# naver/dust3r

Measured on NVIDIA H100. Metric: image-pairs/sec (512x384, ViT-L/B+DPT), higher is better.
Workload: dtype bf16

## Files before the change

dust3r_b200/csrc/attention_wgmma.cu:

```cuda
#include "d3r_common.cuh"
#include "sm90_ptx.cuh"
#include "elementwise.h"
#include "prof.h"
#include "pdl.cuh"

namespace d3r {
namespace attn {

namespace wg {

constexpr int BQ = 128, BK = 128, D = 64;
constexpr int kThreads = 384;
constexpr int kTileBytes = 128 * 64 * 2;
constexpr int kPBytes = 2 * 64 * 128 * 2;
template <bool P_SMEM>
struct Smem {
  static constexpr int kP = P_SMEM ? 2 * kPBytes : 0;
  static constexpr int kBytes = kTileBytes  + 2 * kTileBytes  + 2 * kTileBytes  + kP + 128  + 1024;
  static_assert(kBytes <= 227 * 1024, "shared memory of one CTA");
};

template <bool P_SMEM>
__global__ void __launch_bounds__(kThreads, 1)
attention_kernel(const __grid_constant__ CUtensorMap tmap_q, const __grid_constant__ CUtensorMap tmap_k,
                 const __grid_constant__ CUtensorMap tmap_v, __nv_bfloat16* __restrict__ out, long long ldo, int Nq, int Nk,
                 int heads, int total_tiles, float scale_log2) {
  extern __shared__ uint8_t smem_raw[];
  uint8_t* smem = reinterpret_cast<uint8_t*>((reinterpret_cast<uintptr_t>(smem_raw) + 1023) & ~uintptr_t(1023));
  uint8_t* s_q = smem;
  uint8_t* s_k = s_q + kTileBytes;
  uint8_t* s_v = s_k + 2 * kTileBytes;
  uint8_t* s_p = s_v + 2 * kTileBytes;
  uint64_t* bars = reinterpret_cast<uint64_t*>(s_p + Smem<P_SMEM>::kP);
  uint64_t* q_full = bars + 0;
  uint64_t* q_empty = bars + 1;
  uint64_t* k_full = bars + 2;
  uint64_t* k_empty = bars + 4;
  uint64_t* v_full = bars + 6;
  uint64_t* v_empty = bars + 8;

  const int warp = threadIdx.x >> 5, lane = threadIdx.x & 31;
  const int nq_tiles = (Nq + BQ - 1) / BQ;
  const int nblk = (Nk + BK - 1) / BK;
  auto tile_coords = [&](int t, int& q0, int& h, int& b) {
    q0 = (t % nq_tiles) * BQ;
    h = (t / nq_tiles) % heads;
    b = t / (nq_tiles * heads);
  };

  if (threadIdx.x == 0) {
    ptx::prefetch_tmap(&tmap_q);
    ptx::prefetch_tmap(&tmap_k);
    ptx::prefetch_tmap(&tmap_v);
    ptx::mbar_init(ptx::smem_u32(q_full), 1);
    ptx::mbar_init(ptx::smem_u32(q_empty), 8);
    for (int s = 0; s < 2; ++s) {
      ptx::mbar_init(ptx::smem_u32(&k_full[s]), 1);
      ptx::mbar_init(ptx::smem_u32(&k_empty[s]), 8);
      ptx::mbar_init(ptx::smem_u32(&v_full[s]), 1);
      ptx::mbar_init(ptx::smem_u32(&v_empty[s]), 8);
    }
    ptx::fence_barrier_init();
  }
  __syncthreads();
  pdl::sync_with_predecessor();

  if (warp < 4) {
    ptx::setmaxnreg_dec<24>();
    if (warp == 0 && ptx::elect_one()) {
      uint32_t g = 0, it = 0;
      for (int t = blockIdx.x; t < total_tiles; t += gridDim.x, ++it) {
        int q0, h, b;
        tile_coords(t, q0, h, b);
        ptx::mbar_wait(ptx::smem_u32(q_empty), (it & 1) ^ 1);
        ptx::mbar_arrive_expect_tx(ptx::smem_u32(q_full), kTileBytes);
        ptx::tma_load_3d(ptx::smem_u32(s_q), &tmap_q, ptx::smem_u32(q_full), h * D, q0, b);
        for (int j = 0; j < nblk; ++j, ++g) {
          const int st = g & 1;
          const uint32_t ph = (g >> 1) & 1;
          ptx::mbar_wait(ptx::smem_u32(&k_empty[st]), ph ^ 1);
          ptx::mbar_arrive_expect_tx(ptx::smem_u32(&k_full[st]), kTileBytes);
          ptx::tma_load_3d(ptx::smem_u32(s_k + st * kTileBytes), &tmap_k, ptx::smem_u32(&k_full[st]), h * D, j * BK, b);
          ptx::mbar_wait(ptx::smem_u32(&v_empty[st]), ph ^ 1);
          ptx::mbar_arrive_expect_tx(ptx::smem_u32(&v_full[st]), kTileBytes);
          ptx::tma_load_3d(ptx::smem_u32(s_v + st * kTileBytes), &tmap_v, ptx::smem_u32(&v_full[st]), h * D, j * BK, b);
        }
      }
    }
  } else {
    ptx::setmaxnreg_inc<240>();
    const int cw = (threadIdx.x >> 7) - 1;
    const int wq = warp & 3, q = lane & 3;
    uint8_t* s_pw = s_p + cw * kPBytes;
    uint32_t g = 0, it = 0;
    for (int t = blockIdx.x; t < total_tiles; t += gridDim.x, ++it) {
      int q0, h, b;
      tile_coords(t, q0, h, b);
      float m_run[2] = {-INFINITY, -INFINITY}, l_run[2] = {0.f, 0.f};
      float o[32];
#pragma unroll
      for (int i = 0; i < 32; ++i) o[i] = 0.f;
      ptx::mbar_wait(ptx::smem_u32(q_full), it & 1);
      const uint64_t dq = ptx::desc_kmajor_sw128(ptx::smem_u32(s_q + cw * 64 * 128));
      for (int j = 0; j < nblk; ++j, ++g) {
        const int st = g & 1;
        const uint32_t ph = (g >> 1) & 1;
        float s[64];
        ptx::mbar_wait(ptx::smem_u32(&k_full[st]), ph);
        const uint64_t dk = ptx::desc_kmajor_sw128(ptx::smem_u32(s_k + st * kTileBytes));
        ptx::wgmma_fence();
#pragma unroll
        for (int k = 0; k < D / 16; ++k) ptx::wgmma_m64n128k16_ss(s, dq + uint64_t(2 * k), dk + uint64_t(2 * k), k ? 1u : 0u);
        ptx::wgmma_commit();
        ptx::wgmma_wait<0>();
        ptx::reg_fence(s);
        if (lane == 0) {
          ptx::mbar_arrive(ptx::smem_u32(&k_empty[st]));
          if (j == nblk - 1) ptx::mbar_arrive(ptx::smem_u32(q_empty));
        }
        const int nvalid = Nk - j * BK;
        if (nvalid < BK) {
#pragma unroll
          for (int n = 0; n < 16; ++n)
#pragma unroll
            for (int e = 0; e < 2; ++e)
              if (8 * n + 2 * q + e >= nvalid) { s[4 * n + e] = -INFINITY; s[4 * n + 2 + e] = -INFINITY; }
        }
        float ms[2];
#pragma unroll
        for (int hh = 0; hh < 2; ++hh) {
          float mx = -INFINITY;
#pragma unroll
          for (int n = 0; n < 16; ++n) mx = fmaxf(mx, fmaxf(s[4 * n + 2 * hh], s[4 * n + 2 * hh + 1]));
          mx = fmaxf(mx, __shfl_xor_sync(0xffffffffu, mx, 1));
          mx = fmaxf(mx, __shfl_xor_sync(0xffffffffu, mx, 2));
          const float m_new = fmaxf(m_run[hh], mx);
          const float corr = ptx::ex2_approx((m_run[hh] - m_new) * scale_log2);
          m_run[hh] = m_new;
          l_run[hh] *= corr;
#pragma unroll
          for (int n = 0; n < 8; ++n) { o[4 * n + 2 * hh] *= corr; o[4 * n + 2 * hh + 1] *= corr; }
          ms[hh] = m_new * scale_log2;
        }
        uint32_t pk[32];
#pragma unroll
        for (int n = 0; n < 16; ++n)
#pragma unroll
          for (int hh = 0; hh < 2; ++hh) {
            const float p0 = ptx::ex2_approx(fmaf(s[4 * n + 2 * hh], scale_log2, -ms[hh]));
            const float p1 = ptx::ex2_approx(fmaf(s[4 * n + 2 * hh + 1], scale_log2, -ms[hh]));
            l_run[hh] += p0 + p1;
            pk[2 * n + hh] = pack_bf16x2(p0, p1);
          }
        ptx::mbar_wait(ptx::smem_u32(&v_full[st]), ph);
        const uint32_t sv = ptx::smem_u32(s_v + st * kTileBytes);
        if constexpr (P_SMEM) {
#pragma unroll
          for (int n = 0; n < 16; ++n)
#pragma unroll
            for (int hh = 0; hh < 2; ++hh) {
              const int r = wq * 16 + (lane >> 2) + 8 * hh;
              *reinterpret_cast<uint32_t*>(s_pw + (n >> 3) * (64 * 128) + r * 128 + (((n & 7) ^ (r & 7)) << 4) + 4 * q) = pk[2 * n + hh];
            }
          ptx::fence_proxy_async();
          asm volatile("bar.sync %0, 128;" ::"r"(1 + cw) : "memory");
          const uint32_t sp = ptx::smem_u32(s_pw);
          ptx::wgmma_fence();
#pragma unroll
          for (int kk = 0; kk < BK / 16; ++kk)
            ptx::wgmma_m64n64k16_ss_tb(o, ptx::desc_kmajor_sw128(sp + (kk >> 2) * (64 * 128)) + uint64_t(2 * (kk & 3)),
                                       ptx::desc_mnmajor_sw128(sv + kk * 16 * 128), 1u);
        } else {
          ptx::wgmma_fence();
#pragma unroll
          for (int kk = 0; kk < BK / 16; ++kk) ptx::wgmma_m64n64k16_rs_tb(o, pk + 4 * kk, ptx::desc_mnmajor_sw128(sv + kk * 16 * 128), 1u);
        }
        ptx::wgmma_commit();
        ptx::wgmma_wait<0>();
        ptx::reg_fence(o);
        if constexpr (P_SMEM) asm volatile("bar.sync %0, 128;" ::"r"(1 + cw) : "memory");
        if (lane == 0) ptx::mbar_arrive(ptx::smem_u32(&v_empty[st]));
      }
#pragma unroll
      for (int hh = 0; hh < 2; ++hh) {
        float l = l_run[hh];
        l += __shfl_xor_sync(0xffffffffu, l, 1);
        l += __shfl_xor_sync(0xffffffffu, l, 2);
        const float inv = 1.f / l;
        const int qrow = q0 + cw * 64 + wq * 16 + (lane >> 2) + 8 * hh;
        if (qrow < Nq) {
          __nv_bfloat16* orow = out + ((long long)b * Nq + qrow) * ldo + h * D + 2 * q;
#pragma unroll
          for (int n = 0; n < 8; ++n)
            *reinterpret_cast<uint32_t*>(orow + 8 * n) = pack_bf16x2(o[4 * n + 2 * hh] * inv, o[4 * n + 2 * hh + 1] * inv);
        }
      }
    }
  }
}

}

template <bool P_SMEM>
static int launch_attention(const CUtensorMap& mq, const CUtensorMap& mk, const CUtensorMap& mv, void* out, long long ldo, int B, int heads,
                            int Nq, int Nk, float scale, cudaStream_t st) {
  static unsigned long long attr_devices = 0;
  if (first_launch_on_this_device(attr_devices))
    D3R_CUDA(cudaFuncSetAttribute(wg::attention_kernel<P_SMEM>, cudaFuncAttributeMaxDynamicSharedMemorySize, wg::Smem<P_SMEM>::kBytes));
  const int total_tiles = ((Nq + wg::BQ - 1) / wg::BQ) * heads * B;
  const int slots = num_sms();
  const int rounds = (total_tiles + slots - 1) / slots;
  const int grid = (total_tiles + rounds - 1) / rounds;
  prof::Scope scope(P_SMEM ? "attention_wgmma_psmem" : "attention_wgmma", st, 4.0 * double(B) * heads * double(Nq) * double(Nk) * 64.0);
  D3R_CUDA(pdl::launch(wg::attention_kernel<P_SMEM>, dim3(grid), dim3(wg::kThreads), size_t(wg::Smem<P_SMEM>::kBytes), st, mq, mk, mv,
                       (__nv_bfloat16*)out, ldo, Nq, Nk, heads, total_tiles, scale * 1.4426950408889634f));
  D3R_LAUNCH_CHECK();
  return D3R_OK;
}

static int make_map(CUtensorMap* m, const void* base, long long ld, int cols, int N, int B, int box_rows) {
  const cuuint64_t dims[3] = {(cuuint64_t)cols, (cuuint64_t)N, (cuuint64_t)B};
  const cuuint64_t str[2] = {(cuuint64_t)ld * 2, (cuuint64_t)N * ld * 2};
  const cuuint32_t box[3] = {64, (cuuint32_t)box_rows, 1};
  return encode_tensor_map(m, base, 3, dims, str, box, "attention");
}

static int g_impl = 3;

int attention_hd64(const void* q, long long ldq, const void* k, long long ldk, const void* v, long long ldv, void* out,
                   long long ldo, int B, int heads, int Nq, int Nk, float scale, cudaStream_t st) {
  D3R_CHECK_ARG(q && k && v && out && B > 0 && heads > 0 && Nq > 0 && Nk > 0, "attention: bad arguments");
  D3R_CHECK_ARG(ldq % 8 == 0 && ldk % 8 == 0 && ldv % 8 == 0 && ldo % 8 == 0, "attention: row strides must be multiples of 8");
  D3R_CHECK_ARG(((uintptr_t)q & 15) == 0 && ((uintptr_t)k & 15) == 0 && ((uintptr_t)v & 15) == 0 && ((uintptr_t)out & 15) == 0,
                "attention: pointers must be 16-byte aligned");
  CUtensorMap mq, mk, mv;
  int rc;
  if ((rc = make_map(&mq, q, ldq, heads * 64, Nq, B, wg::BQ))) return rc;
  if ((rc = make_map(&mk, k, ldk, heads * 64, Nk, B, wg::BK))) return rc;
  if ((rc = make_map(&mv, v, ldv, heads * 64, Nk, B, wg::BK))) return rc;
  if (g_impl == 2) return launch_attention<true>(mq, mk, mv, out, ldo, B, heads, Nq, Nk, scale, st);
  return launch_attention<false>(mq, mk, mv, out, ldo, B, heads, Nq, Nk, scale, st);
}

}
}

extern "C" void d3r_set_attention_impl(int32_t impl) { d3r::attn::g_impl = (impl == 2) ? 2 : 3; }

extern "C" int d3r_attention_hd64(const void* q, int64_t ldq, const void* k, int64_t ldk, const void* v, int64_t ldv, void* out,
                                  int64_t ldo, int32_t B, int32_t heads, int32_t Nq, int32_t Nk, float scale, void* stream) {
  return d3r::attn::attention_hd64(q, ldq, k, ldk, v, ldv, out, ldo, B, heads, Nq, Nk, scale, (cudaStream_t)stream);
}
```

dust3r_b200/csrc/sm90_ptx.cuh:

```cuda
#pragma once
#include <cuda.h>
#include <cuda_runtime.h>
#include <cuda_bf16.h>
#include <cstdint>

namespace d3r {
namespace ptx {

__device__ __forceinline__ uint32_t smem_u32(const void* p) { return static_cast<uint32_t>(__cvta_generic_to_shared(p)); }

__device__ __forceinline__ bool elect_one() {
  uint32_t pred = 0;
  asm volatile(
      "{\n"
      ".reg .b32 %%rx;\n"
      ".reg .pred %%px;\n"
      "elect.sync %%rx|%%px, %1;\n"
      "@%%px mov.s32 %0, 1;\n"
      "}\n"
      : "+r"(pred)
      : "r"(0xffffffffu));
  return pred != 0;
}

__device__ __forceinline__ void mbar_init(uint32_t bar, uint32_t count) {
  asm volatile("mbarrier.init.shared::cta.b64 [%0], %1;" ::"r"(bar), "r"(count));
}
__device__ __forceinline__ void fence_barrier_init() { asm volatile("fence.mbarrier_init.release.cluster;" ::: "memory"); }
__device__ __forceinline__ void fence_proxy_async() { asm volatile("fence.proxy.async.shared::cta;" ::: "memory"); }

__device__ __forceinline__ void mbar_arrive_expect_tx(uint32_t bar, uint32_t bytes) {
  asm volatile("mbarrier.arrive.expect_tx.shared::cta.b64 _, [%0], %1;" ::"r"(bar), "r"(bytes) : "memory");
}
__device__ __forceinline__ void mbar_arrive(uint32_t bar) {
  asm volatile("mbarrier.arrive.shared::cta.b64 _, [%0];" ::"r"(bar) : "memory");
}
__device__ __forceinline__ bool mbar_try_wait(uint32_t bar, uint32_t parity) {
  uint32_t done;
  asm volatile(
      "{\n"
      ".reg .pred p;\n"
      "mbarrier.try_wait.parity.shared::cta.b64 p, [%1], %2;\n"
      "selp.u32 %0, 1, 0, p;\n"
      "}\n"
      : "=r"(done)
      : "r"(bar), "r"(parity)
      : "memory");
  return done != 0;
}
__device__ __forceinline__ void mbar_wait(uint32_t bar, uint32_t parity) {
  while (!mbar_try_wait(bar, parity)) {
  }
}
__device__ __forceinline__ void mbar_wait_bounded(uint32_t bar, uint32_t parity) {
  uint32_t spins = 0;
  bool done;
  do {
    done = mbar_try_wait(bar, parity);
    if (!done && ++spins > (1u << 22)) __trap();
  } while (!done);
}

__device__ __forceinline__ void bulk_g2s(uint32_t dst, const void* src, uint32_t bytes, uint32_t bar) {
  asm volatile("cp.async.bulk.shared::cluster.global.mbarrier::complete_tx::bytes [%0], [%1], %2, [%3];"
               ::"r"(dst), "l"(src), "r"(bytes), "r"(bar) : "memory");
}
__device__ __forceinline__ uint64_t policy_evict_first() {
  uint64_t pol;
  asm volatile("createpolicy.fractional.L2::evict_first.b64 %0, 1.0;" : "=l"(pol));
  return pol;
}
__device__ __forceinline__ void bulk_g2s_hint(uint32_t dst, const void* src, uint32_t bytes, uint32_t bar, uint64_t pol) {
  asm volatile("cp.async.bulk.shared::cluster.global.mbarrier::complete_tx::bytes.L2::cache_hint [%0], [%1], %2, [%3], %4;"
               ::"r"(dst), "l"(src), "r"(bytes), "r"(bar), "l"(pol) : "memory");
}

__device__ __forceinline__ void prefetch_tmap(const void* tmap) {
  asm volatile("prefetch.tensormap [%0];" ::"l"(reinterpret_cast<uint64_t>(tmap)) : "memory");
}
__device__ __forceinline__ void tma_load_2d(uint32_t dst, const void* tmap, uint32_t bar, int c0, int c1) {
  asm volatile(
      "cp.async.bulk.tensor.2d.shared::cluster.global.mbarrier::complete_tx::bytes [%0], [%1, {%3, %4}], [%2];"
      ::"r"(dst), "l"(reinterpret_cast<uint64_t>(tmap)), "r"(bar), "r"(c0), "r"(c1)
      : "memory");
}
__device__ __forceinline__ void tma_load_3d(uint32_t dst, const void* tmap, uint32_t bar, int c0, int c1, int c2) {
  asm volatile(
      "cp.async.bulk.tensor.3d.shared::cluster.global.mbarrier::complete_tx::bytes [%0], [%1, {%3, %4, %5}], [%2];"
      ::"r"(dst), "l"(reinterpret_cast<uint64_t>(tmap)), "r"(bar), "r"(c0), "r"(c1), "r"(c2)
      : "memory");
}
__device__ __forceinline__ void tma_load_4d(uint32_t dst, const void* tmap, uint32_t bar, int c0, int c1, int c2, int c3) {
  asm volatile(
      "cp.async.bulk.tensor.4d.shared::cluster.global.mbarrier::complete_tx::bytes [%0], [%1, {%3, %4, %5, %6}], [%2];"
      ::"r"(dst), "l"(reinterpret_cast<uint64_t>(tmap)), "r"(bar), "r"(c0), "r"(c1), "r"(c2), "r"(c3)
      : "memory");
}
__device__ __forceinline__ void tma_load_3d_mc(uint32_t dst, const void* tmap, uint32_t bar, int c0, int c1, int c2, uint16_t mask) {
  asm volatile(
      "cp.async.bulk.tensor.3d.shared::cluster.global.mbarrier::complete_tx::bytes.multicast::cluster [%0], [%1, {%3, %4, %5}], [%2], %6;"
      ::"r"(dst), "l"(reinterpret_cast<uint64_t>(tmap)), "r"(bar), "r"(c0), "r"(c1), "r"(c2), "h"(mask)
      : "memory");
}

__device__ __forceinline__ void tma_store_2d(const void* tmap, uint32_t src, int c0, int c1) {
  asm volatile("cp.async.bulk.tensor.2d.global.shared::cta.tile.bulk_group [%0, {%2, %3}], [%1];"
               ::"l"(reinterpret_cast<uint64_t>(tmap)), "r"(src), "r"(c0), "r"(c1) : "memory");
}
__device__ __forceinline__ void tma_store_4d(const void* tmap, uint32_t src, int c0, int c1, int c2, int c3) {
  asm volatile("cp.async.bulk.tensor.4d.global.shared::cta.tile.bulk_group [%0, {%2, %3, %4, %5}], [%1];"
               ::"l"(reinterpret_cast<uint64_t>(tmap)), "r"(src), "r"(c0), "r"(c1), "r"(c2), "r"(c3) : "memory");
}
__device__ __forceinline__ void tma_reduce_add_2d(const void* tmap, uint32_t src, int c0, int c1) {
  asm volatile("cp.reduce.async.bulk.tensor.2d.global.shared::cta.add.tile.bulk_group [%0, {%2, %3}], [%1];"
               ::"l"(reinterpret_cast<uint64_t>(tmap)), "r"(src), "r"(c0), "r"(c1) : "memory");
}
__device__ __forceinline__ void bulk_commit_group() { asm volatile("cp.async.bulk.commit_group;" ::: "memory"); }
template <int N> __device__ __forceinline__ void bulk_wait_group_read() { asm volatile("cp.async.bulk.wait_group.read %0;" ::"n"(N) : "memory"); }
template <int N> __device__ __forceinline__ void bulk_wait_group() { asm volatile("cp.async.bulk.wait_group %0;" ::"n"(N) : "memory"); }
__device__ __forceinline__ void st_shared_b32(uint32_t addr, uint32_t v) { asm volatile("st.shared.b32 [%0], %1;" ::"r"(addr), "r"(v) : "memory"); }
__device__ __forceinline__ uint32_t ld_shared_b32(uint32_t addr) {
  uint32_t v;
  asm volatile("ld.shared.b32 %0, [%1];" : "=r"(v) : "r"(addr) : "memory");
  return v;
}
__device__ __forceinline__ void st_shared_v2_f32(uint32_t addr, float a, float b) {
  asm volatile("st.shared.v2.f32 [%0], {%1, %2};" ::"r"(addr), "f"(a), "f"(b) : "memory");
}
__device__ __forceinline__ void named_bar_sync(uint32_t id, uint32_t count) { asm volatile("bar.sync %0, %1;" ::"r"(id), "r"(count) : "memory"); }

__device__ __forceinline__ uint32_t cluster_ctarank() {
  uint32_t r;
  asm volatile("mov.u32 %0, %%cluster_ctarank;" : "=r"(r));
  return r;
}
__device__ __forceinline__ void cluster_sync() {
  asm volatile("barrier.cluster.arrive.release.aligned;\nbarrier.cluster.wait.acquire.aligned;" ::: "memory");
}
__device__ __forceinline__ void mbar_arrive_cluster(uint32_t bar, uint32_t rank) {
  asm volatile(
      "{\n"
      ".reg .b32 raddr;\n"
      "mapa.shared::cluster.u32 raddr, %0, %1;\n"
      "mbarrier.arrive.shared::cluster.b64 _, [raddr];\n"
      "}\n" ::"r"(bar), "r"(rank) : "memory");
}

__device__ __forceinline__ float ex2_approx(float x) { float y; asm("ex2.approx.ftz.f32 %0, %1;" : "=f"(y) : "f"(x)); return y; }
__device__ __forceinline__ float rcp_approx(float x) { float y; asm("rcp.approx.ftz.f32 %0, %1;" : "=f"(y) : "f"(x)); return y; }
__device__ __forceinline__ float rsqrt_approx(float x) { float y; asm("rsqrt.approx.ftz.f32 %0, %1;" : "=f"(y) : "f"(x)); return y; }
__device__ __forceinline__ float sqrt_approx(float x) { float y; asm("sqrt.approx.ftz.f32 %0, %1;" : "=f"(y) : "f"(x)); return y; }

template <int N> __device__ __forceinline__ void setmaxnreg_dec() { asm volatile("setmaxnreg.dec.sync.aligned.u32 %0;" ::"n"(N)); }
template <int N> __device__ __forceinline__ void setmaxnreg_inc() { asm volatile("setmaxnreg.inc.sync.aligned.u32 %0;" ::"n"(N)); }

__device__ __forceinline__ void wgmma_fence() { asm volatile("wgmma.fence.sync.aligned;" ::: "memory"); }
__device__ __forceinline__ void wgmma_commit() { asm volatile("wgmma.commit_group.sync.aligned;" ::: "memory"); }
template <int N> __device__ __forceinline__ void wgmma_wait() { asm volatile("wgmma.wait_group.sync.aligned %0;" ::"n"(N) : "memory"); }
template <int N> __device__ __forceinline__ void reg_fence(float (&d)[N]) {
#pragma unroll
  for (int i = 0; i < N; ++i) asm volatile("" : "+f"(d[i])::"memory");
}

__device__ __forceinline__ uint64_t desc_sw128(uint32_t smem_addr, uint32_t lbo_bytes) {
  uint64_t d = 0;
  d |= uint64_t((smem_addr & 0x3FFFF) >> 4);
  d |= uint64_t(lbo_bytes >> 4) << 16;
  d |= uint64_t(1024 >> 4) << 32;
  d |= uint64_t(1) << 62;
  return d;
}
__device__ __forceinline__ uint64_t desc_kmajor_sw128(uint32_t smem_addr) { return desc_sw128(smem_addr, 16); }
__device__ __forceinline__ uint64_t desc_mnmajor_sw128(uint32_t smem_addr) { return desc_sw128(smem_addr, 1024); }

__device__ __forceinline__ void wgmma_m64n64k16_ss(float* d, uint64_t desc_a, uint64_t desc_b, uint32_t accumulate) {
  asm volatile(
      "{\n"
      ".reg .pred p;\n"
      "setp.ne.b32 p, %34, 0;\n"
      "wgmma.mma_async.sync.aligned.m64n64k16.f32.bf16.bf16 "
      "{%0, %1, %2, %3, %4, %5, %6, %7, %8, %9, %10, %11, %12, %13, %14, %15, %16, %17, %18, %19, %20, %21, %22, %23, %24, %25, %26, %27, %28, %29, %30, %31}, %32, %33, p, 1, 1, 0, 0;\n"
      "}\n"
      : "+f"(d[0]), "+f"(d[1]), "+f"(d[2]), "+f"(d[3]), "+f"(d[4]), "+f"(d[5]), "+f"(d[6]), "+f"(d[7]), "+f"(d[8]), "+f"(d[9]), "+f"(d[10]), "+f"(d[11]), "+f"(d[12]), "+f"(d[13]), "+f"(d[14]), "+f"(d[15]), "+f"(d[16]), "+f"(d[17]), "+f"(d[18]), "+f"(d[19]), "+f"(d[20]), "+f"(d[21]), "+f"(d[22]), "+f"(d[23]), "+f"(d[24]), "+f"(d[25]), "+f"(d[26]), "+f"(d[27]), "+f"(d[28]), "+f"(d[29]), "+f"(d[30]), "+f"(d[31])
      : "l"(desc_a), "l"(desc_b), "r"(accumulate));
}
__device__ __forceinline__ void wgmma_m64n128k16_ss(float* d, uint64_t desc_a, uint64_t desc_b, uint32_t accumulate) {
  asm volatile(
      "{\n"
      ".reg .pred p;\n"
      "setp.ne.b32 p, %66, 0;\n"
      "wgmma.mma_async.sync.aligned.m64n128k16.f32.bf16.bf16 "
      "{%0, %1, %2, %3, %4, %5, %6, %7, %8, %9, %10, %11, %12, %13, %14, %15, %16, %17, %18, %19, %20, %21, %22, %23, %24, %25, %26, %27, %28, %29, %30, %31, %32, %33, %34, %35, %36, %37, %38, %39, %40, %41, %42, %43, %44, %45, %46, %47, %48, %49, %50, %51, %52, %53, %54, %55, %56, %57, %58, %59, %60, %61, %62, %63}, %64, %65, p, 1, 1, 0, 0;\n"
      "}\n"
      : "+f"(d[0]), "+f"(d[1]), "+f"(d[2]), "+f"(d[3]), "+f"(d[4]), "+f"(d[5]), "+f"(d[6]), "+f"(d[7]), "+f"(d[8]), "+f"(d[9]), "+f"(d[10]), "+f"(d[11]), "+f"(d[12]), "+f"(d[13]), "+f"(d[14]), "+f"(d[15]), "+f"(d[16]), "+f"(d[17]), "+f"(d[18]), "+f"(d[19]), "+f"(d[20]), "+f"(d[21]), "+f"(d[22]), "+f"(d[23]), "+f"(d[24]), "+f"(d[25]), "+f"(d[26]), "+f"(d[27]), "+f"(d[28]), "+f"(d[29]), "+f"(d[30]), "+f"(d[31]), "+f"(d[32]), "+f"(d[33]), "+f"(d[34]), "+f"(d[35]), "+f"(d[36]), "+f"(d[37]), "+f"(d[38]), "+f"(d[39]), "+f"(d[40]), "+f"(d[41]), "+f"(d[42]), "+f"(d[43]), "+f"(d[44]), "+f"(d[45]), "+f"(d[46]), "+f"(d[47]), "+f"(d[48]), "+f"(d[49]), "+f"(d[50]), "+f"(d[51]), "+f"(d[52]), "+f"(d[53]), "+f"(d[54]), "+f"(d[55]), "+f"(d[56]), "+f"(d[57]), "+f"(d[58]), "+f"(d[59]), "+f"(d[60]), "+f"(d[61]), "+f"(d[62]), "+f"(d[63])
      : "l"(desc_a), "l"(desc_b), "r"(accumulate));
}
__device__ __forceinline__ void wgmma_m64n256k16_ss(float* d, uint64_t desc_a, uint64_t desc_b, uint32_t accumulate) {
  asm volatile(
      "{\n"
      ".reg .pred p;\n"
      "setp.ne.b32 p, %130, 0;\n"
      "wgmma.mma_async.sync.aligned.m64n256k16.f32.bf16.bf16 "
      "{%0, %1, %2, %3, %4, %5, %6, %7, %8, %9, %10, %11, %12, %13, %14, %15, %16, %17, %18, %19, %20, %21, %22, %23, %24, %25, %26, %27, %28, %29, %30, %31, %32, %33, %34, %35, %36, %37, %38, %39, %40, %41, %42, %43, %44, %45, %46, %47, %48, %49, %50, %51, %52, %53, %54, %55, %56, %57, %58, %59, %60, %61, %62, %63, %64, %65, %66, %67, %68, %69, %70, %71, %72, %73, %74, %75, %76, %77, %78, %79, %80, %81, %82, %83, %84, %85, %86, %87, %88, %89, %90, %91, %92, %93, %94, %95, %96, %97, %98, %99, %100, %101, %102, %103, %104, %105, %106, %107, %108, %109, %110, %111, %112, %113, %114, %115, %116, %117, %118, %119, %120, %121, %122, %123, %124, %125, %126, %127}, %128, %129, p, 1, 1, 0, 0;\n"
      "}\n"
      : "+f"(d[0]), "+f"(d[1]), "+f"(d[2]), "+f"(d[3]), "+f"(d[4]), "+f"(d[5]), "+f"(d[6]), "+f"(d[7]), "+f"(d[8]), "+f"(d[9]), "+f"(d[10]), "+f"(d[11]), "+f"(d[12]), "+f"(d[13]), "+f"(d[14]), "+f"(d[15]), "+f"(d[16]), "+f"(d[17]), "+f"(d[18]), "+f"(d[19]), "+f"(d[20]), "+f"(d[21]), "+f"(d[22]), "+f"(d[23]), "+f"(d[24]), "+f"(d[25]), "+f"(d[26]), "+f"(d[27]), "+f"(d[28]), "+f"(d[29]), "+f"(d[30]), "+f"(d[31]), "+f"(d[32]), "+f"(d[33]), "+f"(d[34]), "+f"(d[35]), "+f"(d[36]), "+f"(d[37]), "+f"(d[38]), "+f"(d[39]), "+f"(d[40]), "+f"(d[41]), "+f"(d[42]), "+f"(d[43]), "+f"(d[44]), "+f"(d[45]), "+f"(d[46]), "+f"(d[47]), "+f"(d[48]), "+f"(d[49]), "+f"(d[50]), "+f"(d[51]), "+f"(d[52]), "+f"(d[53]), "+f"(d[54]), "+f"(d[55]), "+f"(d[56]), "+f"(d[57]), "+f"(d[58]), "+f"(d[59]), "+f"(d[60]), "+f"(d[61]), "+f"(d[62]), "+f"(d[63]), "+f"(d[64]), "+f"(d[65]), "+f"(d[66]), "+f"(d[67]), "+f"(d[68]), "+f"(d[69]), "+f"(d[70]), "+f"(d[71]), "+f"(d[72]), "+f"(d[73]), "+f"(d[74]), "+f"(d[75]), "+f"(d[76]), "+f"(d[77]), "+f"(d[78]), "+f"(d[79]), "+f"(d[80]), "+f"(d[81]), "+f"(d[82]), "+f"(d[83]), "+f"(d[84]), "+f"(d[85]), "+f"(d[86]), "+f"(d[87]), "+f"(d[88]), "+f"(d[89]), "+f"(d[90]), "+f"(d[91]), "+f"(d[92]), "+f"(d[93]), "+f"(d[94]), "+f"(d[95]), "+f"(d[96]), "+f"(d[97]), "+f"(d[98]), "+f"(d[99]), "+f"(d[100]), "+f"(d[101]), "+f"(d[102]), "+f"(d[103]), "+f"(d[104]), "+f"(d[105]), "+f"(d[106]), "+f"(d[107]), "+f"(d[108]), "+f"(d[109]), "+f"(d[110]), "+f"(d[111]), "+f"(d[112]), "+f"(d[113]), "+f"(d[114]), "+f"(d[115]), "+f"(d[116]), "+f"(d[117]), "+f"(d[118]), "+f"(d[119]), "+f"(d[120]), "+f"(d[121]), "+f"(d[122]), "+f"(d[123]), "+f"(d[124]), "+f"(d[125]), "+f"(d[126]), "+f"(d[127])
      : "l"(desc_a), "l"(desc_b), "r"(accumulate));
}
__device__ __forceinline__ void wgmma_m64n64k16_rs_tb(float* d, const uint32_t* a, uint64_t desc_b, uint32_t accumulate) {
  asm volatile(
      "{\n"
      ".reg .pred p;\n"
      "setp.ne.b32 p, %37, 0;\n"
      "wgmma.mma_async.sync.aligned.m64n64k16.f32.bf16.bf16 "
      "{%0, %1, %2, %3, %4, %5, %6, %7, %8, %9, %10, %11, %12, %13, %14, %15, %16, %17, %18, %19, %20, %21, %22, %23, %24, %25, %26, %27, %28, %29, %30, %31}, {%32, %33, %34, %35}, %36, p, 1, 1, 1;\n"
      "}\n"
      : "+f"(d[0]), "+f"(d[1]), "+f"(d[2]), "+f"(d[3]), "+f"(d[4]), "+f"(d[5]), "+f"(d[6]), "+f"(d[7]), "+f"(d[8]), "+f"(d[9]), "+f"(d[10]), "+f"(d[11]), "+f"(d[12]), "+f"(d[13]), "+f"(d[14]), "+f"(d[15]), "+f"(d[16]), "+f"(d[17]), "+f"(d[18]), "+f"(d[19]), "+f"(d[20]), "+f"(d[21]), "+f"(d[22]), "+f"(d[23]), "+f"(d[24]), "+f"(d[25]), "+f"(d[26]), "+f"(d[27]), "+f"(d[28]), "+f"(d[29]), "+f"(d[30]), "+f"(d[31])
      : "r"(a[0]), "r"(a[1]), "r"(a[2]), "r"(a[3]), "l"(desc_b), "r"(accumulate));
}
__device__ __forceinline__ void wgmma_m64n64k16_ss_tb(float* d, uint64_t desc_a, uint64_t desc_b, uint32_t accumulate) {
  asm volatile(
      "{\n"
      ".reg .pred p;\n"
      "setp.ne.b32 p, %34, 0;\n"
      "wgmma.mma_async.sync.aligned.m64n64k16.f32.bf16.bf16 "
      "{%0, %1, %2, %3, %4, %5, %6, %7, %8, %9, %10, %11, %12, %13, %14, %15, %16, %17, %18, %19, %20, %21, %22, %23, %24, %25, %26, %27, %28, %29, %30, %31}, %32, %33, p, 1, 1, 0, 1;\n"
      "}\n"
      : "+f"(d[0]), "+f"(d[1]), "+f"(d[2]), "+f"(d[3]), "+f"(d[4]), "+f"(d[5]), "+f"(d[6]), "+f"(d[7]), "+f"(d[8]), "+f"(d[9]), "+f"(d[10]), "+f"(d[11]), "+f"(d[12]), "+f"(d[13]), "+f"(d[14]), "+f"(d[15]), "+f"(d[16]), "+f"(d[17]), "+f"(d[18]), "+f"(d[19]), "+f"(d[20]), "+f"(d[21]), "+f"(d[22]), "+f"(d[23]), "+f"(d[24]), "+f"(d[25]), "+f"(d[26]), "+f"(d[27]), "+f"(d[28]), "+f"(d[29]), "+f"(d[30]), "+f"(d[31])
      : "l"(desc_a), "l"(desc_b), "r"(accumulate));
}

}
}
```

Before: 179.9.

## Rewrite default attention kernel as FA3-style pipeline with three consumer warpgroups

Replaces the default register-P attention kernel with a new warp-specialized kernel. It has one producer warpgroup and three consumer warpgroups covering 192 query rows, a 4-stage K/V pipeline, and double-buffered Q. Consumers take turns issuing WGMMAs through named barriers, and each one overlaps the next QK^T with the current PV product (intra-warpgroup pingpong). Output is written by staging in shared memory and issuing a TMA store. The aim is to hide softmax latency behind tensor-core work and raise throughput. The cost is more complex synchronization and register pressure, and the 192-row tiles may leave a partial tile at the end.

```diff
diff --git a/dust3r_b200/csrc/attention_wgmma.cu b/dust3r_b200/csrc/attention_wgmma.cu
--- a/dust3r_b200/csrc/attention_wgmma.cu
+++ b/dust3r_b200/csrc/attention_wgmma.cu
@@ -13,25 +13,23 @@
 constexpr int kThreads = 384;
 constexpr int kTileBytes = 128 * 64 * 2;
 constexpr int kPBytes = 2 * 64 * 128 * 2;
-template <bool P_SMEM>
-struct Smem {
-  static constexpr int kP = P_SMEM ? 2 * kPBytes : 0;
-  static constexpr int kBytes = kTileBytes  + 2 * kTileBytes  + 2 * kTileBytes  + kP + 128  + 1024;
+
+struct PsmemSmem {
+  static constexpr int kBytes = kTileBytes  + 2 * kTileBytes  + 2 * kTileBytes  + 2 * kPBytes + 128  + 1024;
   static_assert(kBytes <= 227 * 1024, "shared memory of one CTA");
 };
 
-template <bool P_SMEM>
 __global__ void __launch_bounds__(kThreads, 1)
-attention_kernel(const __grid_constant__ CUtensorMap tmap_q, const __grid_constant__ CUtensorMap tmap_k,
-                 const __grid_constant__ CUtensorMap tmap_v, __nv_bfloat16* __restrict__ out, long long ldo, int Nq, int Nk,
-                 int heads, int total_tiles, float scale_log2) {
+attention_psmem_kernel(const __grid_constant__ CUtensorMap tmap_q, const __grid_constant__ CUtensorMap tmap_k,
+                       const __grid_constant__ CUtensorMap tmap_v, __nv_bfloat16* __restrict__ out, long long ldo, int Nq, int Nk,
+                       int heads, int total_tiles, float scale_log2) {
   extern __shared__ uint8_t smem_raw[];
   uint8_t* smem = reinterpret_cast<uint8_t*>((reinterpret_cast<uintptr_t>(smem_raw) + 1023) & ~uintptr_t(1023));
   uint8_t* s_q = smem;
   uint8_t* s_k = s_q + kTileBytes;
   uint8_t* s_v = s_k + 2 * kTileBytes;
   uint8_t* s_p = s_v + 2 * kTileBytes;
-  uint64_t* bars = reinterpret_cast<uint64_t*>(s_p + Smem<P_SMEM>::kP);
+  uint64_t* bars = reinterpret_cast<uint64_t*>(s_p + 2 * kPBytes);
   uint64_t* q_full = bars + 0;
   uint64_t* q_empty = bars + 1;
   uint64_t* k_full = bars + 2;
@@ -154,31 +152,25 @@
           }
         ptx::mbar_wait(ptx::smem_u32(&v_full[st]), ph);
         const uint32_t sv = ptx::smem_u32(s_v + st * kTileBytes);
-        if constexpr (P_SMEM) {
-#pragma unroll
-          for (int n = 0; n < 16; ++n)
-#pragma unroll
-            for (int hh = 0; hh < 2; ++hh) {
-              const int r = wq * 16 + (lane >> 2) + 8 * hh;
-              *reinterpret_cast<uint32_t*>(s_pw + (n >> 3) * (64 * 128) + r * 128 + (((n & 7) ^ (r & 7)) << 4) + 4 * q) = pk[2 * n + hh];
-            }
-          ptx::fence_proxy_async();
-          asm volatile("bar.sync %0, 128;" ::"r"(1 + cw) : "memory");
-          const uint32_t sp = ptx::smem_u32(s_pw);
-          ptx::wgmma_fence();
-#pragma unroll
-          for (int kk = 0; kk < BK / 16; ++kk)
-            ptx::wgmma_m64n64k16_ss_tb(o, ptx::desc_kmajor_sw128(sp + (kk >> 2) * (64 * 128)) + uint64_t(2 * (kk & 3)),
-                                       ptx::desc_mnmajor_sw128(sv + kk * 16 * 128), 1u);
-        } else {
-          ptx::wgmma_fence();
-#pragma unroll
-          for (int kk = 0; kk < BK / 16; ++kk) ptx::wgmma_m64n64k16_rs_tb(o, pk + 4 * kk, ptx::desc_mnmajor_sw128(sv + kk * 16 * 128), 1u);
-        }
+#pragma unroll
+        for (int n = 0; n < 16; ++n)
+#pragma unroll
+          for (int hh = 0; hh < 2; ++hh) {
+            const int r = wq * 16 + (lane >> 2) + 8 * hh;
+            *reinterpret_cast<uint32_t*>(s_pw + (n >> 3) * (64 * 128) + r * 128 + (((n & 7) ^ (r & 7)) << 4) + 4 * q) = pk[2 * n + hh];
+          }
+        ptx::fence_proxy_async();
+        asm volatile("bar.sync %0, 128;" ::"r"(1 + cw) : "memory");
+        const uint32_t sp = ptx::smem_u32(s_pw);
+        ptx::wgmma_fence();
+#pragma unroll
+        for (int kk = 0; kk < BK / 16; ++kk)
+          ptx::wgmma_m64n64k16_ss_tb(o, ptx::desc_kmajor_sw128(sp + (kk >> 2) * (64 * 128)) + uint64_t(2 * (kk & 3)),
+                                     ptx::desc_mnmajor_sw128(sv + kk * 16 * 128), 1u);
         ptx::wgmma_commit();
         ptx::wgmma_wait<0>();
         ptx::reg_fence(o);
-        if constexpr (P_SMEM) asm volatile("bar.sync %0, 128;" ::"r"(1 + cw) : "memory");
+        asm volatile("bar.sync %0, 128;" ::"r"(1 + cw) : "memory");
         if (lane == 0) ptx::mbar_arrive(ptx::smem_u32(&v_empty[st]));
       }
 #pragma unroll
@@ -199,23 +191,234 @@
   }
 }
 
-}
-
-template <bool P_SMEM>
-static int launch_attention(const CUtensorMap& mq, const CUtensorMap& mk, const CUtensorMap& mv, void* out, long long ldo, int B, int heads,
-                            int Nq, int Nk, float scale, cudaStream_t st) {
-  static unsigned long long attr_devices = 0;
-  if (first_launch_on_this_device(attr_devices))
-    D3R_CUDA(cudaFuncSetAttribute(wg::attention_kernel<P_SMEM>, cudaFuncAttributeMaxDynamicSharedMemorySize, wg::Smem<P_SMEM>::kBytes));
-  const int total_tiles = ((Nq + wg::BQ - 1) / wg::BQ) * heads * B;
-  const int slots = num_sms();
-  const int rounds = (total_tiles + slots - 1) / slots;
-  const int grid = (total_tiles + rounds - 1) / rounds;
-  prof::Scope scope(P_SMEM ? "attention_wgmma_psmem" : "attention_wgmma", st, 4.0 * double(B) * heads * double(Nq) * double(Nk) * 64.0);
-  D3R_CUDA(pdl::launch(wg::attention_kernel<P_SMEM>, dim3(grid), dim3(wg::kThreads), size_t(wg::Smem<P_SMEM>::kBytes), st, mq, mk, mv,
-                       (__nv_bfloat16*)out, ldo, Nq, Nk, heads, total_tiles, scale * 1.4426950408889634f));
-  D3R_LAUNCH_CHECK();
-  return D3R_OK;
+constexpr int kConsumers = 3;
+constexpr int kQRows = 64 * kConsumers;
+constexpr int kQBytes = kQRows * 128;
+constexpr int kPipeThreads = 128 * (1 + kConsumers);
+constexpr int kConsumerRegs = ((65536 / 128 - 24) / kConsumers) / 8 * 8;
+constexpr int kStages = 4;
+constexpr int kOBytes = 64 * 64 * 2;
+struct Smem {
+  static constexpr int kBytes = 2 * kQBytes  + 2 * kStages * kTileBytes  + kConsumers * kOBytes  +
+                                256  + 1024;
+  static_assert(kBytes <= 227 * 1024, "shared memory of one CTA");
+};
+constexpr uint32_t kBarTurn = 1;
+constexpr uint32_t kBarEpi = 1 + kConsumers;
+static_assert(kBarEpi + kConsumers <= 16, "named barriers");
+
+__global__ void __launch_bounds__(kPipeThreads, 1)
+attention_kernel(const __grid_constant__ CUtensorMap tmap_q, const __grid_constant__ CUtensorMap tmap_k,
+                 const __grid_constant__ CUtensorMap tmap_v, const __grid_constant__ CUtensorMap tmap_o, int Nq, int Nk, int heads,
+                 int total_tiles, float scale_log2) {
+  extern __shared__ uint8_t smem_raw[];
+  uint8_t* smem = reinterpret_cast<uint8_t*>((reinterpret_cast<uintptr_t>(smem_raw) + 1023) & ~uintptr_t(1023));
+  uint8_t* s_q = smem;
+  uint8_t* s_k = s_q + 2 * kQBytes;
+  uint8_t* s_v = s_k + kStages * kTileBytes;
+  uint8_t* s_o = s_v + kStages * kTileBytes;
+  uint64_t* bars = reinterpret_cast<uint64_t*>(s_o + kConsumers * kOBytes);
+  uint64_t* q_full = bars;
+  uint64_t* q_empty = bars + 2;
+  uint64_t* k_full = bars + 4;
+  uint64_t* k_empty = k_full + kStages;
+  uint64_t* v_full = k_empty + kStages;
+  uint64_t* v_empty = v_full + kStages;
+
+  const int warp = threadIdx.x >> 5, lane = threadIdx.x & 31;
+  const int nq_tiles = (Nq + kQRows - 1) / kQRows;
+  const int nblk = (Nk + BK - 1) / BK;
+  auto tile_coords = [&](int t, int& q0, int& h, int& b) {
+    q0 = (t % nq_tiles) * kQRows;
+    h = (t / nq_tiles) % heads;
+    b = t / (nq_tiles * heads);
+  };
+
+  if (threadIdx.x == 0) {
+    ptx::prefetch_tmap(&tmap_q);
+    ptx::prefetch_tmap(&tmap_k);
+    ptx::prefetch_tmap(&tmap_v);
+    ptx::prefetch_tmap(&tmap_o);
+    for (int s = 0; s < 2; ++s) {
+      ptx::mbar_init(ptx::smem_u32(&q_full[s]), 1);
+      ptx::mbar_init(ptx::smem_u32(&q_empty[s]), 4 * kConsumers);
+    }
+    for (int s = 0; s < kStages; ++s) {
+      ptx::mbar_init(ptx::smem_u32(&k_full[s]), 1);
+      ptx::mbar_init(ptx::smem_u32(&k_empty[s]), 4 * kConsumers);
+      ptx::mbar_init(ptx::smem_u32(&v_full[s]), 1);
+      ptx::mbar_init(ptx::smem_u32(&v_empty[s]), 4 * kConsumers);
+    }
+    ptx::fence_barrier_init();
+  }
+  __syncthreads();
+  pdl::sync_with_predecessor();
+
+  if (warp < 4) {
+    ptx::setmaxnreg_dec<24>();
+    if (warp == 0 && ptx::elect_one()) {
+      uint32_t st = 0, ph = 0, it = 0;
+      for (int t = blockIdx.x; t < total_tiles; t += gridDim.x, ++it) {
+        int q0, h, b;
+        tile_coords(t, q0, h, b);
+        const uint32_t qs = it & 1;
+        ptx::mbar_wait(ptx::smem_u32(&q_empty[qs]), ((it >> 1) & 1) ^ 1);
+        ptx::mbar_arrive_expect_tx(ptx::smem_u32(&q_full[qs]), kQBytes);
+        ptx::tma_load_3d(ptx::smem_u32(s_q + qs * kQBytes), &tmap_q, ptx::smem_u32(&q_full[qs]), h * D, q0, b);
+        for (int j = 0; j < nblk; ++j) {
+          ptx::mbar_wait(ptx::smem_u32(&k_empty[st]), ph ^ 1);
+          ptx::mbar_arrive_expect_tx(ptx::smem_u32(&k_full[st]), kTileBytes);
+          ptx::tma_load_3d(ptx::smem_u32(s_k + st * kTileBytes), &tmap_k, ptx::smem_u32(&k_full[st]), h * D, j * BK, b);
+          ptx::mbar_wait(ptx::smem_u32(&v_empty[st]), ph ^ 1);
+          ptx::mbar_arrive_expect_tx(ptx::smem_u32(&v_full[st]), kTileBytes);
+          ptx::tma_load_3d(ptx::smem_u32(s_v + st * kTileBytes), &tmap_v, ptx::smem_u32(&v_full[st]), h * D, j * BK, b);
+          if (++st == kStages) { st = 0; ph ^= 1; }
+        }
+      }
+    }
+  } else {
+    ptx::setmaxnreg_inc<kConsumerRegs>();
+    const int cw = (threadIdx.x >> 7) - 1;
+    const int wq = warp & 3, q = lane & 3;
+    const bool store_thread = (threadIdx.x & 127) == 0;
+    const uint32_t so = ptx::smem_u32(s_o + cw * kOBytes);
+    const uint32_t my_turn = kBarTurn + cw, next_turn = kBarTurn + (cw + 1) % kConsumers;
+    if (cw == kConsumers - 1) ptx::named_bar_arrive(kBarTurn, 256);
+    uint32_t st = 0, ph = 0, it = 0;
+    for (int t = blockIdx.x; t < total_tiles; t += gridDim.x, ++it) {
+      int q0, h, b;
+      tile_coords(t, q0, h, b);
+      float m_run[2] = {-INFINITY, -INFINITY}, l_run[2] = {0.f, 0.f};
+      float o[32];
+#pragma unroll
+      for (int i = 0; i < 32; ++i) o[i] = 0.f;
+      const uint32_t qs = it & 1;
+      ptx::mbar_wait(ptx::smem_u32(&q_full[qs]), (it >> 1) & 1);
+      const uint64_t dq = ptx::desc_kmajor_sw128(ptx::smem_u32(s_q + qs * kQBytes + cw * 64 * 128));
+      float s[64];
+      uint32_t pk[32];
+      float corr[2];
+      uint32_t pst = 0, pph = 0;
+      auto issue_s = [&] {
+        ptx::mbar_wait(ptx::smem_u32(&k_full[st]), ph);
+        const uint64_t dk = ptx::desc_kmajor_sw128(ptx::smem_u32(s_k + st * kTileBytes));
+        ptx::wgmma_fence();
+#pragma unroll
+        for (int k = 0; k < D / 16; ++k) ptx::wgmma_m64n128k16_ss(s, dq + uint64_t(2 * k), dk + uint64_t(2 * k), k ? 1u : 0u);
+        ptx::wgmma_commit();
+      };
+      auto issue_pv = [&] {
+        const uint32_t sv = ptx::smem_u32(s_v + pst * kTileBytes);
+        ptx::wgmma_fence();
+#pragma unroll
+        for (int kk = 0; kk < BK / 16; ++kk) ptx::wgmma_m64n64k16_rs_tb(o, pk + 4 * kk, ptx::desc_mnmajor_sw128(sv + kk * 16 * 128), 1u);
+        ptx::wgmma_commit();
+      };
+      auto softmax = [&](int j) {
+        if (lane == 0) {
+          ptx::mbar_arrive(ptx::smem_u32(&k_empty[st]));
+          if (j == nblk - 1) ptx::mbar_arrive(ptx::smem_u32(&q_empty[qs]));
+        }
+        const int nvalid = Nk - j * BK;
+        if (nvalid < BK) {
+#pragma unroll
+          for (int n = 0; n < 16; ++n)
+#pragma unroll
+            for (int e = 0; e < 2; ++e)
+              if (8 * n + 2 * q + e >= nvalid) { s[4 * n + e] = -INFINITY; s[4 * n + 2 + e] = -INFINITY; }
+        }
+        float ms[2];
+#pragma unroll
+        for (int hh = 0; hh < 2; ++hh) {
+          float mx = -INFINITY;
+#pragma unroll
+          for (int n = 0; n < 16; ++n) mx = fmaxf(mx, fmaxf(s[4 * n + 2 * hh], s[4 * n + 2 * hh + 1]));
+          mx = fmaxf(mx, __shfl_xor_sync(0xffffffffu, mx, 1));
+          mx = fmaxf(mx, __shfl_xor_sync(0xffffffffu, mx, 2));
+          const float m_new = fmaxf(m_run[hh], mx);
+          corr[hh] = ptx::ex2_approx((m_run[hh] - m_new) * scale_log2);
+          m_run[hh] = m_new;
+          l_run[hh] *= corr[hh];
+          ms[hh] = m_new * scale_log2;
+        }
+#pragma unroll
+        for (int n = 0; n < 16; ++n)
+#pragma unroll
+          for (int hh = 0; hh < 2; ++hh) {
+            const float p0 = ptx::ex2_approx(fmaf(s[4 * n + 2 * hh], scale_log2, -ms[hh]));
+            const float p1 = ptx::ex2_approx(fmaf(s[4 * n + 2 * hh + 1], scale_log2, -ms[hh]));
+            l_run[hh] += p0 + p1;
+            s[4 * n + 2 * hh] = p0;
+            s[4 * n + 2 * hh + 1] = p1;
+          }
+      };
+      auto rescale_pack = [&] {
+#pragma unroll
+        for (int hh = 0; hh < 2; ++hh)
+#pragma unroll
+          for (int n = 0; n < 8; ++n) { o[4 * n + 2 * hh] *= corr[hh]; o[4 * n + 2 * hh + 1] *= corr[hh]; }
+#pragma unroll
+        for (int n = 0; n < 16; ++n)
+#pragma unroll
+          for (int hh = 0; hh < 2; ++hh) pk[2 * n + hh] = pack_bf16x2(s[4 * n + 2 * hh], s[4 * n + 2 * hh + 1]);
+        pst = st;
+        pph = ph;
+        if (++st == kStages) { st = 0; ph ^= 1; }
+      };
+      ptx::named_bar_sync(my_turn, 256);
+      issue_s();
+      ptx::named_bar_arrive(next_turn, 256);
+      ptx::wgmma_wait<0>();
+      ptx::reg_fence(s);
+      softmax(0);
+      rescale_pack();
+      for (int j = 1; j < nblk; ++j) {
+        ptx::mbar_wait(ptx::smem_u32(&v_full[pst]), pph);
+        ptx::named_bar_sync(my_turn, 256);
+        issue_s();
+        issue_pv();
+        ptx::named_bar_arrive(next_turn, 256);
+        ptx::wgmma_wait<1>();
+        ptx::reg_fence(s);
+        softmax(j);
+        ptx::wgmma_wait<0>();
+        ptx::reg_fence(o);
+        if (lane == 0) ptx::mbar_arrive(ptx::smem_u32(&v_empty[pst]));
+        rescale_pack();
+      }
+      ptx::mbar_wait(ptx::smem_u32(&v_full[pst]), pph);
+      ptx::named_bar_sync(my_turn, 256);
+      issue_pv();
+      ptx::named_bar_arrive(next_turn, 256);
+      ptx::wgmma_wait<0>();
+      ptx::reg_fence(o);
+      if (lane == 0) ptx::mbar_arrive(ptx::smem_u32(&v_empty[pst]));
+      if (store_thread) ptx::bulk_wait_group_read<0>();
+      ptx::named_bar_sync(kBarEpi + cw, 128);
+#pragma unroll
+      for (int hh = 0; hh < 2; ++hh) {
+        float l = l_run[hh];
+        l += __shfl_xor_sync(0xffffffffu, l, 1);
+        l += __shfl_xor_sync(0xffffffffu, l, 2);
+        const float inv = 1.f / l;
+        const int r = wq * 16 + (lane >> 2) + 8 * hh;
+#pragma unroll
+        for (int n = 0; n < 8; ++n)
+          ptx::st_shared_b32(so + r * 128 + ((n ^ (r & 7)) << 4) + 4 * q,
+                             pack_bf16x2(o[4 * n + 2 * hh] * inv, o[4 * n + 2 * hh + 1] * inv));
+      }
+      ptx::fence_proxy_async();
+      ptx::named_bar_sync(kBarEpi + cw, 128);
+      if (store_thread && q0 + 64 * cw < Nq) {
+        ptx::tma_store_3d(&tmap_o, so, h * D, q0 + 64 * cw, b);
+        ptx::bulk_commit_group();
+      }
+    }
+    if (store_thread) ptx::bulk_wait_group<0>();
+    if (cw == 0) ptx::named_bar_sync(kBarTurn, 256);
+  }
+}
+
 }
 
 static int make_map(CUtensorMap* m, const void* base, long long ld, int cols, int N, int B, int box_rows) {
@@ -223,6 +426,43 @@
   const cuuint64_t str[2] = {(cuuint64_t)ld * 2, (cuuint64_t)N * ld * 2};
   const cuuint32_t box[3] = {64, (cuuint32_t)box_rows, 1};
   return encode_tensor_map(m, base, 3, dims, str, box, "attention");
+}
+
+static void launch_shape(int B, int heads, int Nq, int tile_rows, int& total_tiles, int& grid) {
+  total_tiles = ((Nq + tile_rows - 1) / tile_rows) * heads * B;
+  const int slots = num_sms();
+  const int rounds = (total_tiles + slots - 1) / slots;
+  grid = (total_tiles + rounds - 1) / rounds;
+}
+
+static double flops(int B, int heads, int Nq, int Nk) { return 4.0 * double(B) * heads * double(Nq) * double(Nk) * 64.0; }
+
+static int launch_attention(const CUtensorMap& mq, const CUtensorMap& mk, const CUtensorMap& mv, const CUtensorMap& mo, int B,
+                            int heads, int Nq, int Nk, float scale, cudaStream_t st) {
+  static unsigned long long attr_devices = 0;
+  if (first_launch_on_this_device(attr_devices))
+    D3R_CUDA(cudaFuncSetAttribute(wg::attention_kernel, cudaFuncAttributeMaxDynamicSharedMemorySize, wg::Smem::kBytes));
+  int total_tiles, grid;
+  launch_shape(B, heads, Nq, wg::kQRows, total_tiles, grid);
+  prof::Scope scope("attention_wgmma", st, flops(B, heads, Nq, Nk));
+  D3R_CUDA(pdl::launch(wg::attention_kernel, dim3(grid), dim3(wg::kPipeThreads), size_t(wg::Smem::kBytes), st, mq, mk, mv, mo, Nq, Nk,
+                       heads, total_tiles, scale * 1.4426950408889634f));
+  D3R_LAUNCH_CHECK();
+  return D3R_OK;
+}
+
+static int launch_attention_psmem(const CUtensorMap& mq, const CUtensorMap& mk, const CUtensorMap& mv, void* out, long long ldo, int B,
+                                  int heads, int Nq, int Nk, float scale, cudaStream_t st) {
+  static unsigned long long attr_devices = 0;
+  if (first_launch_on_this_device(attr_devices))
+    D3R_CUDA(cudaFuncSetAttribute(wg::attention_psmem_kernel, cudaFuncAttributeMaxDynamicSharedMemorySize, wg::PsmemSmem::kBytes));
+  int total_tiles, grid;
+  launch_shape(B, heads, Nq, wg::BQ, total_tiles, grid);
+  prof::Scope scope("attention_wgmma_psmem", st, flops(B, heads, Nq, Nk));
+  D3R_CUDA(pdl::launch(wg::attention_psmem_kernel, dim3(grid), dim3(wg::kThreads), size_t(wg::PsmemSmem::kBytes), st, mq, mk, mv,
+                       (__nv_bfloat16*)out, ldo, Nq, Nk, heads, total_tiles, scale * 1.4426950408889634f));
+  D3R_LAUNCH_CHECK();
+  return D3R_OK;
 }
 
 static int g_impl = 3;
@@ -233,13 +473,15 @@
   D3R_CHECK_ARG(ldq % 8 == 0 && ldk % 8 == 0 && ldv % 8 == 0 && ldo % 8 == 0, "attention: row strides must be multiples of 8");
   D3R_CHECK_ARG(((uintptr_t)q & 15) == 0 && ((uintptr_t)k & 15) == 0 && ((uintptr_t)v & 15) == 0 && ((uintptr_t)out & 15) == 0,
                 "attention: pointers must be 16-byte aligned");
-  CUtensorMap mq, mk, mv;
+  CUtensorMap mq, mk, mv, mo;
   int rc;
-  if ((rc = make_map(&mq, q, ldq, heads * 64, Nq, B, wg::BQ))) return rc;
+  const bool psmem = g_impl == 2;
+  if ((rc = make_map(&mq, q, ldq, heads * 64, Nq, B, psmem ? wg::BQ : wg::kQRows))) return rc;
   if ((rc = make_map(&mk, k, ldk, heads * 64, Nk, B, wg::BK))) return rc;
   if ((rc = make_map(&mv, v, ldv, heads * 64, Nk, B, wg::BK))) return rc;
-  if (g_impl == 2) return launch_attention<true>(mq, mk, mv, out, ldo, B, heads, Nq, Nk, scale, st);
-  return launch_attention<false>(mq, mk, mv, out, ldo, B, heads, Nq, Nk, scale, st);
+  if (psmem) return launch_attention_psmem(mq, mk, mv, out, ldo, B, heads, Nq, Nk, scale, st);
+  if ((rc = make_map(&mo, out, ldo, heads * 64, Nq, B, 64))) return rc;
+  return launch_attention(mq, mk, mv, mo, B, heads, Nq, Nk, scale, st);
 }
 
 }
diff --git a/dust3r_b200/csrc/sm90_ptx.cuh b/dust3r_b200/csrc/sm90_ptx.cuh
--- a/dust3r_b200/csrc/sm90_ptx.cuh
+++ b/dust3r_b200/csrc/sm90_ptx.cuh
@@ -106,6 +106,10 @@
 __device__ __forceinline__ void tma_store_2d(const void* tmap, uint32_t src, int c0, int c1) {
   asm volatile("cp.async.bulk.tensor.2d.global.shared::cta.tile.bulk_group [%0, {%2, %3}], [%1];"
                ::"l"(reinterpret_cast<uint64_t>(tmap)), "r"(src), "r"(c0), "r"(c1) : "memory");
+}
+__device__ __forceinline__ void tma_store_3d(const void* tmap, uint32_t src, int c0, int c1, int c2) {
+  asm volatile("cp.async.bulk.tensor.3d.global.shared::cta.tile.bulk_group [%0, {%2, %3, %4}], [%1];"
+               ::"l"(reinterpret_cast<uint64_t>(tmap)), "r"(src), "r"(c0), "r"(c1), "r"(c2) : "memory");
 }
 __device__ __forceinline__ void tma_store_4d(const void* tmap, uint32_t src, int c0, int c1, int c2, int c3) {
   asm volatile("cp.async.bulk.tensor.4d.global.shared::cta.tile.bulk_group [%0, {%2, %3, %4, %5}], [%1];"
@@ -128,6 +132,7 @@
   asm volatile("st.shared.v2.f32 [%0], {%1, %2};" ::"r"(addr), "f"(a), "f"(b) : "memory");
 }
 __device__ __forceinline__ void named_bar_sync(uint32_t id, uint32_t count) { asm volatile("bar.sync %0, %1;" ::"r"(id), "r"(count) : "memory"); }
+__device__ __forceinline__ void named_bar_arrive(uint32_t id, uint32_t count) { asm volatile("bar.arrive %0, %1;" ::"r"(id), "r"(count) : "memory"); }
 
 __device__ __forceinline__ uint32_t cluster_ctarank() {
   uint32_t r;
```

Result: faster. 184.2 (median of 6 runs) (+2.4%).
